# leggedrobotics/art_planner

Hardware: NVIDIA H100
Metric: pose-validity checks/s (higher is better)
Workload: dtype f32

## Files before the change

### art_planner_b200/capi.py

```python
from __future__ import annotations

import ctypes as C
import os

HERE = os.path.dirname(os.path.abspath(__file__))
LIB_PATH = os.path.join(HERE, "libartp.so")

ARTP_OK, ARTP_E_INVALID, ARTP_E_NOMAP, ARTP_E_CUDA, ARTP_E_LIMIT, ARTP_E_NOWEIGHTS, ARTP_E_WINDOW = 0, -1, -2, -3, -4, -5, -6


class ArtpError(RuntimeError):
    def __init__(self, code: int, msg: str):
        super().__init__(f"artp error {code}: {msg}")
        self.code = code


class ArtpParams(C.Structure):
    _fields_ = [(n, C.c_double) for n in (
        "torso_length", "torso_width", "torso_height", "torso_off_x", "torso_off_y", "torso_off_z",
        "feet_off_x", "feet_off_y", "feet_off_z", "reach_x", "reach_y", "reach_z")] + [
        ("unknown_space_untraversable", C.c_int), ("use_directional_cost", C.c_int),
        ("max_lon_vel", C.c_double), ("max_lat_vel", C.c_double), ("max_ang_vel", C.c_double),
        ("cost_w_energy", C.c_float), ("cost_w_time", C.c_float), ("cost_w_risk", C.c_float),
        ("risk_threshold", C.c_float), ("device", C.c_int)]
# ... 60 lines not shown
                ("sample_from_distribution", C.c_int), ("use_inverse_vertex_density", C.c_int),
                ("use_max_prob_unknown_samples", C.c_int), ("max_prob_unknown_samples", C.c_double), ("basic", ArtpBasicParams),
                ("simplify", C.c_int), ("clear_roadmap", C.c_int), ("seed", C.c_uint64)]


class ArtpPlanInfo(C.Structure):
    _fields_ = [("status", C.c_int32), ("sampled", C.c_int32)] + [(n, C.c_uint64) for n in (
        "first_sample", "draws_used", "start_draw", "goal_draw", "simplify_seed", "n_vertices", "n_edges")] + [
        ("solve", ArtpRoadmapSolveInfo), ("path_cost", C.c_double), ("simplify", ArtpSimplifyInfo)] + [
        (n, C.c_int32) for n in ("goal_clipped", "goal_inside", "start_index", "goal_index")] + [
        (n, C.c_double * 7) for n in ("goal_clipped_state", "goal_projected", "start_repaired", "goal_repaired")] + [
        (n, C.c_float) for n in ("ms_sample_graph", "ms_update_edges", "ms_endpoints", "ms_solve", "ms_simplify")] + [
        ("host_syncs", C.c_uint32), ("bytes_h2d", C.c_uint64), ("bytes_d2h", C.c_uint64)]


class ArtpPlannerMapInfo(C.Structure):
    _fields_ = [("host_syncs", C.c_uint32), ("bytes_h2d", C.c_uint64), ("bytes_d2h", C.c_uint64)]


class ArtpStats(C.Structure):
    _fields_ = [("poses_checked", C.c_uint64), ("poses_deferred", C.c_uint64), ("kernel_launches", C.c_uint64),
                ("last_deferred", C.c_uint32), ("last_launches", C.c_uint32), ("last_queued_boxes", C.c_uint32),
                ("last_queued_warp_stage", C.c_uint32), ("last_queued_reach_stage", C.c_uint32),
                ("last_reach_plane_stage", C.c_uint32)]


_lib = None


def load():
    global _lib
    if _lib is not None:
        return _lib
    if not os.path.exists(LIB_PATH):
        raise FileNotFoundError(f"{LIB_PATH} not built; run `python -m art_planner_b200.build` (needs nvcc)")
    lib = C.CDLL(LIB_PATH)
    vp, sz, i32, dbl = C.c_void_p, C.c_size_t, C.c_int, C.c_double
    lib.artp_create.argtypes = [C.POINTER(ArtpParams), C.POINTER(vp)]
    lib.artp_destroy.argtypes = [vp]
    lib.artp_destroy.restype = None
    lib.artp_last_error.argtypes = [vp]
    lib.artp_last_error.restype = C.c_char_p
    lib.artp_set_map.argtypes = [vp, vp, vp, i32, i32, dbl, dbl, dbl]
    lib.artp_has_map.argtypes = [vp]
    lib.artp_check_poses.argtypes = [vp, vp, sz, vp]
    lib.artp_check_poses_device.argtypes = [vp, vp, sz, vp, vp]
    lib.artp_check_poses_f32.argtypes = [vp, vp, sz, vp]
# ... 38 lines not shown
    lib.artp_update_sample_distribution_device.argtypes = [vp, C.POINTER(ArtpSampleDistributionParams), vp, sz, vp]
    lib.artp_debug_gaussian_kernel.argtypes = [i32, dbl, vp]
    lib.artp_roadmap_clear.argtypes = [vp, sz, sz]
    lib.artp_roadmap_add_milestones.argtypes = [vp, vp, sz]
    lib.artp_roadmap_sample_graph.argtypes = [vp, C.POINTER(ArtpRoadmapParams), C.POINTER(ArtpSampleDistributionParams), u64, u64,
                                              C.POINTER(u64)]
    lib.artp_roadmap_get.argtypes = [vp, sz, vp, vp, sz, vp, C.POINTER(sz), C.POINTER(sz)]
    lib.artp_roadmap_update_edges.argtypes = [vp]
    lib.artp_roadmap_solve.argtypes = [vp, vp, vp, C.POINTER(ArtpSe3Space), vp, sz, C.POINTER(sz), C.POINTER(dbl),
                                       C.POINTER(ArtpRoadmapSolveInfo)]
    lib.artp_roadmap_get_edge_costs.argtypes = [vp, sz, vp, vp, C.POINTER(sz)]
    lib.artp_debug_se3_ops.argtypes = [vp, vp, vp, vp, sz, vp, vp]
    lib.artp_simplify_path.argtypes = [vp, vp, sz, C.POINTER(ArtpSe3Space), i32, dbl, u64, vp, sz, C.POINTER(sz),
                                       C.POINTER(ArtpSimplifyInfo)]
    lib.artp_planner_set_map.argtypes = [vp, C.POINTER(ArtpPlannerParams), vp, vp, vp, vp, i32, i32, dbl, dbl, dbl,
                                         C.POINTER(ArtpPlannerMapInfo)]
    lib.artp_planner_get_space.argtypes = [vp, C.POINTER(ArtpSe3Space)]
    lib.artp_plan.argtypes = [vp, C.POINTER(ArtpPlannerParams), vp, vp, vp, sz, C.POINTER(sz), C.POINTER(ArtpPlanInfo)]
    lib.artp_host_alloc.restype = C.c_void_p
    lib.artp_host_alloc.argtypes = [sz]
    lib.artp_host_free.argtypes = [vp]
    lib.artp_debug_set_group_capacity.argtypes = [vp, i32]
    lib.artp_debug_get_reach_queue.argtypes = [vp, vp, sz, C.POINTER(sz)]
    lib.artp_set_timing.argtypes = [vp, i32]
    lib.artp_get_last_timing.argtypes = [vp, C.POINTER(C.c_float)]
    lib.artp_get_last_stage_timing.argtypes = [vp, C.POINTER(C.c_float)]
    lib.artp_version.restype = C.c_char_p
    lib.artp_cost_weights_size.restype = C.c_size_t
    lib.artp_cost_weights_size_for.restype = C.c_size_t
    lib.artp_cost_weights_size_for.argtypes = [i32]
    lib.artp_set_cost_weights.argtypes = [vp, vp, sz]
    lib.artp_get_cost_network.argtypes = [vp, C.POINTER(i32)]
    lib.artp_update_features.argtypes = [vp]
    lib.artp_motion_cost.argtypes = [vp, vp, sz, vp]
    lib.artp_motion_cost_device.argtypes = [vp, vp, sz, vp, vp]
    lib.artp_combine_cost.argtypes = [vp, vp, sz, vp, vp]
    lib.artp_motion_cost_split.argtypes = [vp, vp, vp, sz, dbl, vp]
    lib.artp_motion_cost_split_device.argtypes = [vp, vp, vp, sz, vp, sz, vp, vp, vp, vp]
    lib.artp_get_features.argtypes = [vp, vp, sz, C.POINTER(i32), C.POINTER(i32)]
    lib.artp_set_cnn_mode.argtypes = [vp, i32]
    lib.artp_get_cnn_timing.argtypes = [vp, C.POINTER(C.c_float)]
    _lib = lib
    return lib


def make_params(rp, device: int = 0, cost_weights=(0.0, 1.0, 5.0), risk_threshold=0.5) -> ArtpParams:
# ... 37 lines not shown
```

### art_planner_b200/checker.py

```python
from __future__ import annotations

import ctypes as C

import numpy as np

from . import capi


def _is_torch_cuda(x) -> bool:
    return hasattr(x, "is_cuda") and bool(x.is_cuda)


class _Handle:

    def __init__(self, robot_params, device: int = 0, cost_weights=(0.0, 1.0, 5.0), risk_threshold=0.5):
        self.lib = capi.load()
        self.params = robot_params
        self.device = device
        p = capi.make_params(robot_params, device, cost_weights, risk_threshold)
        h = C.c_void_p()
        rc = self.lib.artp_create(C.byref(p), C.byref(h))
        if rc != 0:
            raise capi.ArtpError(rc, self.lib.artp_last_error(None).decode())
        self.h = h
# ... 239 lines not shown
        if out_cnt is None:
            out_cnt = torch.empty(1, dtype=torch.int32, device=bits.device)
        self._h.check(self._h.lib.artp_compact_bits_device(self._h.h, C.c_void_p(bits.data_ptr()), n, int(base),
                                                           C.c_void_p(out_idx.data_ptr()), C.c_void_p(out_cnt.data_ptr()),
                                                           _stream_ptr()))
        return out_idx, out_cnt

    def setMode(self, mode: int) -> None:
        self._h.check(self._h.lib.artp_set_mode(self._h.h, int(mode)))

    def pollError(self) -> None:
        self._h.check(self._h.lib.artp_poll_error(self._h.h))

    def debugSetGroupCapacity(self, max_triangles: int) -> None:
        self._h.check(self._h.lib.artp_debug_set_group_capacity(self._h.h, int(max_triangles)))

    def debugReachQueue(self):
        import numpy as np
        n = C.c_size_t(0)
        self._h.check(self._h.lib.artp_debug_get_reach_queue(self._h.h, None, 0, C.byref(n)))
        buf = np.empty((n.value, 20), dtype=np.uint32)
        self._h.check(self._h.lib.artp_debug_get_reach_queue(self._h.h, C.c_void_p(buf.ctypes.data), n.value, C.byref(n)))
        return buf[:, 14:18].view(np.int32).copy(), buf[:, 19].copy()

    def stats(self) -> dict:
        return self._h.stats()

    def setTiming(self, enable: bool) -> None:
        self._h.check(self._h.lib.artp_set_timing(self._h.h, int(bool(enable))))

    def lastKernelTimesMs(self):
        ms = (C.c_float * 3)()
        self._h.check(self._h.lib.artp_get_last_timing(self._h.h, ms))
        return float(ms[0]), float(ms[1]), float(ms[2])

    def lastStageTimesMs(self):
        ms = (C.c_float * 5)()
        self._h.check(self._h.lib.artp_get_last_stage_timing(self._h.h, ms))
        return tuple(float(x) for x in ms)

    @property
    def handle(self) -> _Handle:
        return self._h


class SE3FromSE2Sampler:
# ... 579 lines not shown
```

### art_planner_b200/csrc/artp_capi.cu

```cuda
#include <cassert>
#include <climits>
#include <cmath>
#include <cstdlib>
#include <cstring>
#include <cudaTypedefs.h>
#include <type_traits>
#include <vector>

#include "artp_internal.h"
#include "artp_kernels.cuh"
#include "artp_tiles.cuh"

namespace artp_api {

constexpr int kMaxSlices = 9;

struct QueueCtr { uint32_t end, claim; };
struct alignas(32) BoxQueues { QueueCtr big, reach, group; };
struct Counters { BoxQueues q; uint32_t defer; };

struct Shape { int grid = 0, block = 0, smem = 0; };

struct Pipeline {
  enum { kBig, kReach, kGroup };
  Counters* d_ctr = nullptr;
  artp::BoxRec* recs[3] = {};
  uint32_t* d_defer = nullptr;
  size_t recs_cap = 0;
  BoxQueues* d_slices = nullptr;
  unsigned long long* d_compact_state = nullptr;
  size_t compact_state_cap = 0;
  uint32_t compact_epoch = 0;
  artp::TileCfg tile_cfg[2] = {};
  CUtensorMap tile_map[2][2];
  Shape tile[2];
  Shape groups;
  Shape grouping;
  int tcap = 0;
  int tcap_override = 0;
  int mode = 0;
  uint8_t* h_small_out = nullptr;
  bool deferred_unread = false;
  cudaStream_t streams[4] = {};
  cudaStream_t& copy_stream = streams[0];
  cudaStream_t& box_stream = streams[1];
  cudaStream_t& group_stream = streams[2];
  cudaStream_t& tile_stream = streams[3];
  cudaEvent_t order_ev[2 * kMaxSlices + 3] = {};
  cudaEvent_t *const copy_ev = order_ev, *const slice_ev = order_ev + kMaxSlices;
  cudaEvent_t& box_ev = order_ev[2 * kMaxSlices];
  cudaEvent_t &group_ev = order_ev[2 * kMaxSlices + 1], &tile_ev = order_ev[2 * kMaxSlices + 2];
// ... 279 lines not shown
  const size_t need = 5 * std::min(n_items, kChunkItems);
  if (h->pipe->recs_cap >= need) return ARTP_OK;
  const size_t cap = std::max<size_t>(need, 1u << 16);
  h->pipe->recs_cap = 0;
  for (artp::BoxRec*& r : h->pipe->recs) { size_t had = 0; TRY(grow(h, r, had, cap)); }
  size_t had = 0;
  TRY(grow(h, h->pipe->d_defer, had, cap));
  h->pipe->recs_cap = cap;
  return ARTP_OK;
}

struct HostFeed {
  const char* host;
  char* dev;
  size_t bytes_per_item;
  size_t slice_items;
  float schedule[8];
};
constexpr size_t kScheduleItems = 1u << 18;
constexpr int kPipeReachCtasPerSm = 2;

__global__ void close_slice_kernel(const BoxQueues* round, BoxQueues* slices, int i) {
  const BoxQueues prev = i ? slices[i - 1] : BoxQueues{};
  slices[i].group = {round->group.end, prev.group.end};
  slices[i].reach = {round->reach.end, prev.reach.end};
  slices[i].big = {round->big.end, prev.big.end};
}

artp::Work items(artp::Work w, size_t lo, size_t hi) {
  w.item_base = (uint32_t)lo;
  w.n_items = (uint32_t)hi;
  return w;
}
int launch_classify(Handle* h, const artp::Work& w, size_t lo, size_t hi, BoxQueues* q, cudaStream_t s) {
  const Pipeline& p = *h->pipe;
  return launch(h, artp::classify_items_kernel, (unsigned)((hi - lo + artp::kClassifyItems - 1) / artp::kClassifyItems),
                artp::kClassifyItems, 0, s, h->chk, items(w, lo, hi), p.recs[p.kBig], p.recs[p.kReach],
                p.groups.grid ? p.recs[p.kGroup] : nullptr, &q->big.end, &q->reach.end, &q->group.end, p.mode == 1);
}

int launch_big_tile(Handle* h, const artp::Work& w, size_t lo, size_t hi, BoxQueues* q, cudaStream_t s) {
  Pipeline& p = *h->pipe;
  const int wpc = p.tile[0].block / 32;
  const unsigned grid = (unsigned)std::min<size_t>((size_t)p.tile[0].grid, (5 * (hi - lo) + wpc - 1) / wpc);
  return launch(h, artp::box_tiles_warp_kernel, grid, p.tile[0].block, p.tile[0].smem, s, h->chk, p.tile_map[0][0],
                p.tile_map[0][1], p.tile_cfg[0], items(w, lo, hi), p.recs[p.kBig], &q->big.end, &q->big.claim, &p.d_ctr->defer,
                p.d_defer, 0u, p.mode == 1);
}
int launch_reach_warp(Handle* h, const artp::Work& w, size_t lo, size_t hi, BoxQueues* q, cudaStream_t s, unsigned reach_cap) {
  if (!h->chk.reach_tw) return ARTP_OK;
  Pipeline& p = *h->pipe;
  const int wpc = p.tile[1].block / 32;
  const unsigned grid = (unsigned)std::min<size_t>({(size_t)p.tile[1].grid, (4 * (hi - lo) + wpc - 1) / wpc, reach_cap});
  return launch(h, artp::box_tiles_warp_kernel, grid, p.tile[1].block, p.tile[1].smem, s, h->chk, p.tile_map[1][1],
                p.tile_map[1][1], p.tile_cfg[1], items(w, lo, hi), p.recs[p.kReach], &q->reach.end, &q->reach.claim,
                &p.d_ctr->defer, p.d_defer, artp::kDeferReachBit, p.mode == 1);
}
int launch_reach_groups(Handle* h, const artp::Work& w, size_t lo, size_t hi, BoxQueues* q, cudaStream_t s, unsigned reach_cap) {
  const Pipeline& p = *h->pipe;
  if (!p.groups.grid) return ARTP_OK;
  const unsigned grid = (unsigned)std::min<size_t>({(size_t)p.groups.grid, (hi - lo + 7) / 8, reach_cap});
  return launch(h, artp::reach_groups_kernel, grid, p.groups.block, p.groups.smem, s, h->chk, p.tile_map[1][1], p.tile_cfg[1],
                items(w, lo, hi), p.recs[p.kGroup], &q->group.end, &q->group.claim);
}

int launch_grouping(Handle* h, const artp::Work& w, size_t lo, size_t hi, cudaStream_t s) {
  const Pipeline& p = *h->pipe;
  const unsigned grid = (unsigned)std::min<size_t>((size_t)p.grouping.grid, 5 * (hi - lo));
  return launch(h, artp::box_items_block_kernel, grid, p.grouping.block, p.grouping.smem, s, h->chk, items(w, lo, hi),
                p.recs[p.kBig], p.recs[p.kReach], &p.d_ctr->defer, p.d_defer, p.tcap, h->d_err);
}

int run_round_device(Handle* h, const artp::Work& w, cudaStream_t s, size_t base, size_t end, bool timed) {
  Pipeline& p = *h->pipe;
  CU_TRY(h, cudaMemsetAsync(p.d_ctr, 0, sizeof(Counters), s));
  if (timed) CU_TRY(h, cudaEventRecord(p.ev[0], s));
  BoxQueues* q = &p.d_ctr->q;
  TRY(launch_classify(h, w, base, end, q, s));
  if (timed) CU_TRY(h, cudaEventRecord(p.ev[1], s));
  const bool fork = !p.timing && h->chk.reach_tw;
  if (fork) {
    CU_TRY(h, cudaEventRecord(p.slice_ev[0], s));
    CU_TRY(h, cudaStreamWaitEvent(p.tile_stream, p.slice_ev[0], 0));
    CU_TRY(h, cudaStreamWaitEvent(p.box_stream, p.slice_ev[0], 0));
    if (p.groups.grid) CU_TRY(h, cudaStreamWaitEvent(p.group_stream, p.slice_ev[0], 0));
  }
// ... 451 lines not shown
  LOCK_HANDLE(h, hh);
  return timed_round_ms(h, ms5, {{0, 1}, {1, 2}, {2, 3}, {3, 4}, {4, 5}});
}

void* artp_host_alloc(size_t bytes) {
  void* p = nullptr;
  if (bytes == 0 || cudaHostAlloc(&p, bytes, cudaHostAllocPortable) != cudaSuccess) return nullptr;
  return p;
}
void artp_host_free(void* p) { if (p) cudaFreeHost(p); }

int artp_poll_error(artp_handle* hh) {
  LOCK_HANDLE(h, hh);
  return take_sticky_error(h);
}

int artp_debug_set_group_capacity(artp_handle* hh, int max_triangles) {
  LOCK_HANDLE(h, hh);
  if (max_triangles < 0) return ARTP_E_INVALID;
  h->pipe->tcap_override = max_triangles;
  return ARTP_OK;
}

int artp_debug_get_reach_queue(artp_handle* hh, void* recs, size_t cap, size_t* n) {
  LOCK_HANDLE(h, hh);
  if (!n || (cap && !recs)) return ARTP_E_INVALID;
  CU_TRY(h, cudaSetDevice(h->device));
  Counters ctr{};
  CU_TRY(h, cudaMemcpy(&ctr, h->pipe->d_ctr, sizeof(ctr), cudaMemcpyDeviceToHost));
  *n = ctr.q.reach.end;
  const size_t k = std::min(cap, (size_t)ctr.q.reach.end);
  if (k) CU_TRY(h, cudaMemcpy(recs, h->pipe->recs[h->pipe->kReach], k * sizeof(artp::BoxRec), cudaMemcpyDeviceToHost));
  return ARTP_OK;
}

int artp_get_stats(artp_handle* hh, artp_stats* out) {
  LOCK_HANDLE(h, hh);
  if (!out) return ARTP_E_INVALID;
  CU_TRY(h, cudaSetDevice(h->device));
  Counters ctr{};
  CU_TRY(h, cudaMemcpy(&ctr, h->pipe->d_ctr, sizeof(ctr), cudaMemcpyDeviceToHost));
  h->stats.last_deferred = ctr.defer;
  h->stats.last_queued_boxes = ctr.q.big.end + ctr.q.reach.end + ctr.q.group.end;
  h->stats.last_queued_warp_stage = ctr.q.big.end;
  h->stats.last_queued_reach_stage = ctr.q.reach.end;
  h->stats.last_reach_plane_stage = ctr.q.group.end;
  if (h->pipe->deferred_unread) { h->stats.poses_deferred += ctr.defer; h->pipe->deferred_unread = false; }
  *out = h->stats;
  return take_sticky_error(h);
}

int artp_set_map(artp_handle* hh, const float* elevation, const float* elevation_masked, int rows, int cols, double res,
                 double cx, double cy) {
  return artp_set_map_window(hh, elevation, elevation_masked, rows, cols, res, cx, cy, 0, rows);
}

int artp_set_map_window(artp_handle* hh, const float* elevation, const float* elevation_masked, int rows, int cols, double res,
                        double cx, double cy, int row0, int nrows) {
  LOCK_CALL(h, hh);
  h->planner_map = false;
  return upload_map(h, elevation, elevation_masked, false, rows, cols, res, cx, cy, row0, nrows);
}

}

int artp_api::upload_map(Handle* h, const float* elevation, const float* elevation_masked, bool device_src, int rows, int cols,
                         double res, double cx, double cy, int row0, int nrows) {
  if (!elevation || !elevation_masked || rows < 2 || cols < 2 || !(res > 0)) { h->err = "bad map arguments"; return ARTP_E_INVALID; }
  if (row0 < 0 || nrows < 2 || row0 + nrows > rows || (row0 & 3)) {
// ... 278 lines not shown
```

### art_planner_b200/csrc/artp_kernels.cuh

```cuda
#pragma once

#include "artp_device.cuh"

namespace artp {

constexpr int kWarpsPerCta = 8;
constexpr int kMaxCand = 32;
constexpr int kBloomWords = 128;
constexpr unsigned kFull = 0xffffffffu;

enum { R_FREE = 0, R_HIT = 1, R_DEFER = 2 };

__device__ __forceinline__ bool box_fails(bool foot, int r) { return foot ? r == R_FREE : r == R_HIT; }

struct WarpScratch {
  float cpl[kMaxCand][4];
  int cidx[kMaxCand];
  uint32_t bloom[kBloomWords];
  uint32_t bloom2[kBloomWords];
  uint32_t cand_bits[kBloomWords];
};

struct Work {
  const double* s1 = nullptr;
// ... 650 lines not shown
  fl = (uint32_t)k;
  const int g = box_geometry(c, R, R1, t, k, b);
  if (g != -1) return g;
  const int r = zone_classify(c, b, k, force_all, fl);
  return (r == -1 && probe_applies(b, fl) && vertex_probe(c, b, k > 0)) ? R_HIT : r;
}

constexpr int kClassifyItems = 64;
constexpr int kClassifyWarps = kClassifyItems / 32;
constexpr int kPoseWords = 21;
enum { PEND_BIG = 1, PEND_REACH = 2, PEND_GROUP = 3 };

struct ClassifyShared {
  float pose[kPoseWords][kClassifyItems];
  float probe_f[4][kClassifyItems];
  int probe_i[4][kClassifyItems];
  uint8_t valid[kClassifyItems];
  uint8_t pend[5][kClassifyItems];
  uint16_t live[kClassifyItems];
  uint16_t probe[kClassifyItems];
  uint16_t emit[5 * kClassifyItems];
  unsigned long long warp_sum[kClassifyWarps];
  int warp_count[kClassifyWarps];
  uint32_t base[3];
};
static_assert(kClassifyItems <= 256, "emit packs the item index into 8 bits");

__device__ __forceinline__ void load_pose(const ClassifyShared& s, int i, float t[3], float R[9], float R1[9]) {
#pragma unroll
  for (int j = 0; j < 3; ++j) t[j] = s.pose[j][i];
#pragma unroll
  for (int j = 0; j < 9; ++j) { R[j] = s.pose[3 + j][i]; R1[j] = s.pose[12 + j][i]; }
}

__device__ __forceinline__ unsigned long long cta_scan(ClassifyShared& s, unsigned long long v, unsigned long long& total) {
  const int lane = threadIdx.x & 31, wid = threadIdx.x >> 5;
  unsigned long long incl = v;
#pragma unroll
  for (int o = 1; o < 32; o <<= 1) {
    const unsigned long long y = __shfl_up_sync(kFull, incl, o);
    if (lane >= o) incl += y;
  }
  if (lane == 31) s.warp_sum[wid] = incl;
  __syncthreads();
  unsigned long long before = 0;
  total = 0;
#pragma unroll
  for (int q = 0; q < kClassifyWarps; ++q) {
    const unsigned long long x = s.warp_sum[q];
// ... 2 lines not shown
  }
  return before + incl - v;
}

__device__ __forceinline__ int cta_compact(ClassifyShared& s, uint16_t* list, bool pred, int entry) {
  const int lane = threadIdx.x & 31, wid = threadIdx.x >> 5;
  const unsigned m = __ballot_sync(kFull, pred);
  if (lane == 0) s.warp_count[wid] = __popc(m);
  __syncthreads();
  int before = 0, total = 0;
#pragma unroll
  for (int q = 0; q < kClassifyWarps; ++q) {
    const int x = s.warp_count[q];
    before += q < wid ? x : 0;
    total += x;
  }
  if (pred) list[before + __popc(m & ((1u << lane) - 1u))] = (uint16_t)entry;
  __syncthreads();
  return total;
}

__global__ void __launch_bounds__(kClassifyItems, 16)
classify_items_kernel(const Checker c, const Work w, BoxRec* __restrict__ recs_w, BoxRec* __restrict__ recs_f,
                      BoxRec* __restrict__ recs_g, uint32_t* __restrict__ count_w, uint32_t* __restrict__ count_f,
                      uint32_t* __restrict__ count_g, int force_all) {
  __shared__ ClassifyShared s;
  const int tid = threadIdx.x;
  const uint32_t item0 = w.item_base + blockIdx.x * kClassifyItems;
  const bool in_range = item0 + tid < w.n_items;
  if (in_range) {
    double st[7];
    load_item_state(w, item0 + tid, st);
    float t[3], R[9], Rb[9];
    pose3_from_se3(st, t, R);
#pragma unroll
    for (int i = 0; i < 9; ++i) Rb[i] = R[i];
    orthogonalize_r(Rb);
#pragma unroll
    for (int j = 0; j < 3; ++j) s.pose[j][tid] = t[j];
#pragma unroll
    for (int j = 0; j < 9; ++j) s.pose[3 + j][tid] = R[j];
#pragma unroll
    for (int j = 0; j < 3; ++j) { s.pose[12 + j][tid] = -Rb[j]; s.pose[15 + j][tid] = Rb[6 + j]; s.pose[18 + j][tid] = Rb[3 + j]; }
  }
  s.valid[tid] = in_range ? 1 : 0;
#pragma unroll
  for (int k = 0; k < 5; ++k) s.pend[k][tid] = 0;

// ... 29 lines not shown
    if (!foot) break;
    const int n_probe = cta_compact(s, s.probe, probe, tid);
    if (tid < n_probe) {
      const int p = s.probe[tid], i = s.live[p];
      BoxCtx b;
      b.P[0] = s.probe_f[0][p]; b.P[1] = s.probe_f[1][p]; b.P[2] = s.probe_f[2][p]; b.minB = s.probe_f[3][p];
      b.x0 = s.probe_i[0][p]; b.x1 = s.probe_i[1][p]; b.z0 = s.probe_i[2][p]; b.z1 = s.probe_i[3][p];
#pragma unroll
      for (int j = 0; j < 9; ++j) b.R1[j] = s.pose[12 + j][i];
      b.side[0] = c.side[1][0]; b.side[1] = c.side[1][1]; b.side[2] = c.side[1][2];
      if (vertex_probe(c, b, true)) s.pend[k][i] = 0;
    }
  }
  __syncthreads();

  const bool valid = s.valid[tid] != 0;
  if (in_range) {
    const uint32_t slot = item_slot(w, item0 + tid);
    if (w.edge_mode) { if (!valid) w.valid[slot] = 0; }
    else w.valid[slot] = (uint8_t)valid;
  }
  unsigned long long cnt = 0;
  if (valid) {
#pragma unroll
    for (int k = 0; k < 5; ++k) {
      const int q = s.pend[k][tid] >> 6;
      if (q) cnt += 1ull << (21 * (q - 1));
    }
  }
  unsigned long long tot;
  unsigned long long off = cta_scan(s, cnt, tot);
  if (tot == 0) return;
  const uint32_t n_w = (uint32_t)(tot & 0x1FFFFF), n_f = (uint32_t)((tot >> 21) & 0x1FFFFF), n_g = (uint32_t)(tot >> 42);
  if (tid == 0) {
    s.base[0] = n_w ? atomicAdd(count_w, n_w) : 0u;
    s.base[1] = n_f ? atomicAdd(count_f, n_f) : 0u;
    s.base[2] = n_g ? atomicAdd(count_g, n_g) : 0u;
  }
  if (cnt) {
    uint32_t pw = (uint32_t)(off & 0x1FFFFF), pf = n_w + (uint32_t)((off >> 21) & 0x1FFFFF), pg = n_w + n_f + (uint32_t)(off >> 42);
#pragma unroll
    for (int k = 0; k < 5; ++k) {
      const int q = s.pend[k][tid] >> 6;
      const uint16_t e = (uint16_t)((k << 8) | tid);
      if (q == PEND_BIG) s.emit[pw++] = e;
      else if (q == PEND_REACH) s.emit[pf++] = e;
      else if (q == PEND_GROUP) s.emit[pg++] = e;
    }
  }
  __syncthreads();
  const uint32_t n_rec = n_w + n_f + n_g;
#pragma unroll 1
  for (uint32_t j = tid; j < n_rec; j += kClassifyItems) {
    const int e = s.emit[j], i = e & 0xFF, k = e >> 8;
    float t[3], R[9], R1[9];
    load_pose(s, i, t, R, R1);
    BoxCtx b;
    box_geometry(c, R, R1, t, k, b);
    BoxRec o;
#pragma unroll
    for (int m = 0; m < 9; ++m) o.R1[m] = R1[m];
    o.P[0] = b.P[0]; o.P[1] = b.P[1]; o.P[2] = b.P[2];
    o.minB = b.minB; o.maxB = b.maxB;
    o.x0 = b.x0; o.x1 = b.x1; o.z0 = b.z0; o.z1 = b.z1;
    o.item = item_slot(w, item0 + i);
    o.flags = s.pend[k][i] & 0x3Fu;
    if (j < n_w) recs_w[s.base[0] + j] = o;
    else if (j < n_w + n_f) recs_f[s.base[1] + (j - n_w)] = o;
    else recs_g[s.base[2] + (j - n_w - n_f)] = o;
  }
}

struct BlockShared {
  float* planes;
  int* group;
  uint8_t* state;
  int T_cap;
};
__device__ __forceinline__ BlockShared block_shared(unsigned char* smem, int T_cap) {
  BlockShared sh;
  sh.T_cap = T_cap;
  sh.planes = reinterpret_cast<float*>(smem);
  sh.group = reinterpret_cast<int*>(smem + (size_t)T_cap * 16);
  sh.state = reinterpret_cast<uint8_t*>(smem + (size_t)T_cap * 20);
  return sh;
}

__device__ __forceinline__ float block_reduce_max(float v, float* red, bool is_max) {
  const int lane = threadIdx.x & 31, wid = threadIdx.x >> 5;
#pragma unroll
  for (int o = 16; o > 0; o >>= 1) {
    const float a = __shfl_xor_sync(kFull, v, o);
// ... 245 lines not shown
```

### art_planner_b200/csrc/artp_tiles.cuh

```cuda
#pragma once

#include <cuda.h>

#include "artp_kernels.cuh"

namespace artp {

constexpr uint32_t kDeferReachBit = 0x80000000u;
constexpr int kTileChunk = 8;

__device__ __forceinline__ uint32_t smem_addr(const void* p) { return (uint32_t)__cvta_generic_to_shared(p); }
__device__ __forceinline__ void mbar_init(uint64_t* bar, uint32_t count) {
  asm volatile("mbarrier.init.shared::cta.b64 [%0], %1;" ::"r"(smem_addr(bar)), "r"(count));
}
__device__ __forceinline__ void mbar_expect_tx(uint64_t* bar, uint32_t bytes) {
  asm volatile("mbarrier.arrive.expect_tx.shared::cta.b64 _, [%0], %1;" ::"r"(smem_addr(bar)), "r"(bytes) : "memory");
}
__device__ __forceinline__ void mbar_wait(uint64_t* bar, uint32_t parity) {
  asm volatile(
      "{\n\t"
      ".reg .pred P1;\n\t"
      "TWAIT_LOOP:\n\t"
      "mbarrier.try_wait.parity.shared::cta.b64 P1, [%0], %1;\n\t"
      "@P1 bra TWAIT_DONE;\n\t"
// ... 81 lines not shown
      phase[slot] ^= 1u;
      if (dead) continue;
      BoxCtx b;
      rec_to_ctx(c, r, b);
      int res;
      if ((b.x1 - b.x0) + 4 > tc.tw || (b.z1 - b.z0) + 1 > tc.th) {
        res = R_DEFER;
      } else {
        const ZoneView zv{reinterpret_cast<const float*>(slots + (size_t)slot * tc.stride) + (b.x0 & 3), tc.tw};
        res = box_collide_warp<true>(foot ? c.f[1] : c.f[0], b, zv, ws, lane, c.cell_margin, (r.flags & REC_NEEDS_REDUCE) != 0,
                                     (r.flags & REC_ALLFINITE) != 0, (r.flags & REC_MERGEFREE) != 0);
      }
      if (lane == 0) {
        if (res == R_DEFER) defer_list[atomicAdd(defer_count, 1u)] = ri | queue_bit;
        else if (box_fails(foot, res)) w.valid[slot_item] = 0;
      }
    }
  }
}

constexpr int kGroupRounds = 8;
constexpr int kGroupTasks = 64;

__global__ void __launch_bounds__(kMaxTileWarps * 32, 3)
reach_groups_kernel(const Checker c, const __grid_constant__ CUtensorMap map1, const TileCfg tc, const Work w,
                    const BoxRec* __restrict__ recs, const uint32_t* __restrict__ rec_count, uint32_t* __restrict__ work_counter) {
  extern __shared__ __align__(128) unsigned char tile_smem[];
  __shared__ uint64_t bars[kMaxTileWarps][2];
  __shared__ uint16_t tasks_all[kMaxTileWarps][4][kGroupTasks];
  __shared__ __align__(16) float ctx_all[kMaxTileWarps][4][16];
  const int lane = threadIdx.x & 31, wid = threadIdx.x >> 5, g = lane >> 3, gl = lane & 7;
  const Field& f = c.f[1];
  unsigned char* slots = warp_tile_slots(tile_smem, tc, 8, bars[wid]);
  uint16_t* tasks = tasks_all[wid][g];
  uint32_t phase = 0u;
  const uint32_t total = *rec_count;
  const unsigned gshift = (unsigned)g * 8u;
  auto prefetch = [&](uint32_t first, int slot) {
    const uint32_t ri = first + (uint32_t)g;
    int x0 = 0, z0 = 0;
    const bool act = ri < total;
    if (act && gl == 0) { x0 = rec_x0(recs + ri); z0 = rec_z0(recs + ri); }
    const int nact = (int)min(4u, total - first);
    if (lane == 0) mbar_expect_tx(&bars[wid][slot], (uint32_t)nact * tc.bytes);
#pragma unroll 1
    for (int q = 0; q < nact; ++q) {
      const int sx = __shfl_sync(kFull, x0, q * 8), sz = __shfl_sync(kFull, z0, q * 8);
      if (lane == 0) tma_tile_2d(slots + (size_t)(slot * 4 + q) * tc.stride, &map1, &bars[wid][slot], (sx & ~3) - tc.x_off, sz);
    }
  };
  const uint32_t nwarps8 = 8u * gridDim.x * (blockDim.x >> 5);
  uint32_t next_r0 = 0, next_n = 0;
  auto claim = [&]() {
    if (lane == 0) {
      const uint32_t cur = *(volatile const uint32_t*)work_counter;
      next_n = 4u * (cur < total ? min(max((total - cur) / nwarps8, 1u), (uint32_t)kGroupRounds) : 1u);
      next_r0 = atomicAdd(work_counter, next_n);
    }
  };
  claim();
  for (;;) {
    const uint32_t r0 = __shfl_sync(kFull, next_r0, 0), nclaim = __shfl_sync(kFull, next_n, 0);
    if (r0 >= total) break;
    claim();
    const int nrounds = (int)((min(r0 + nclaim, total) - r0 + 3u) / 4u);
    __syncwarp();
    prefetch(r0, 0);
#pragma unroll 1
    for (int round = 0; round < nrounds; ++round) {
      const int slot = round & 1;
      const uint32_t ri = r0 + 4u * (uint32_t)round + (uint32_t)g;
      const bool act = ri < total;
      BoxRec r = {};
      if (act) r = load_rec(recs + ri);
      if (round + 1 < nrounds) { __syncwarp(); prefetch(r0 + 4u * (uint32_t)(round + 1), slot ^ 1); }
      int alive = 0;
      if (act && gl == 0) alive = (*(volatile const uint8_t*)(w.valid + r.item) != 0);
      alive = __shfl_sync(kFull, alive, 0, 8);
      mbar_wait(&bars[wid][slot], (phase >> slot) & 1u);
      phase ^= 1u << slot;
      __syncwarp();
      bool gdone = !(act && alive);
      BoxCtx b;
      rec_to_ctx(c, r, b);
      if (gdone) { b.x0 = b.z0 = 0; b.x1 = b.z1 = 1; }
      if (gl == 0) {
        float* cx = ctx_all[wid][g];
#pragma unroll
        for (int i = 0; i < 9; ++i) cx[i] = b.R1[i];
        cx[9] = b.P[0]; cx[10] = b.P[1]; cx[11] = b.P[2]; cx[12] = b.minB;
        cx[13] = __int_as_float(b.x0); cx[14] = __int_as_float(b.z0);
      }
      const float* tile = reinterpret_cast<const float*>(slots + (size_t)(slot * 4 + g) * tc.stride) + (b.x0 & 3);
      const float top = b.maxB + (1e-4f + 4e-6f * fabsf(b.maxB));
      bool ghit = false;
      const bool allFinite = (r.flags & REC_ALLFINITE) != 0;
      {
        const float xr = box_half_extent(b.R1, b.side, 0) + 1e-4f, zr = box_half_extent(b.R1, b.side, 2) + 1e-4f;
        const int vx0 = max(b.x0, (int)ceilf((b.P[0] - xr) * f.iW)), vx1 = min(b.x1, (int)floorf((b.P[0] + xr) * f.iW));
        const int vz0 = max(b.z0, (int)ceilf((b.P[2] - zr) * f.iD)), vz1 = min(b.z1, (int)floorf((b.P[2] + zr) * f.iD));
        const int nXi = max(vx1 - vx0 + 1, 0), nZi = max(vz1 - vz0 + 1, 0), nVi = nXi * nZi;
// ... 73 lines not shown
            const int lx = tk >> 9, lz = (tk >> 1) & 0xff, ccx = tx0 + lx, ccz = tz0 + lz;
            const float* p = reinterpret_cast<const float*>(slots + (size_t)(slot * 4 + gi) * tc.stride) + (tx0 & 3) + lz * tc.tw + lx;
            const float hA = p[0], hB = p[1], hC = p[tc.tw], hD = p[tc.tw + 1];
            if (tri_kept(isUp, hA, hB, hC, hD, tb.minB)) {
              float pl[4], cxs[4], czs[4];
              cell_plane(f, isUp, ccx, ccz, hA, hB, hC, hD, pl);
              const int nc = box_plane(tb, pl, 4, cxs, czs);
              const int tcx = isUp ? ccx : ccx + 1, tcz = isUp ? ccz : ccz + 1;
              bool hit = false;
#pragma unroll
              for (int i = 0; i < 4; ++i) hit = hit || (i < nc && on_tri(f, isUp, tcx, tcz, cxs[i], czs[i]));
              if (hit) hit_groups |= 1u << gi;
            }
          }
        }
        __syncwarp();
        hit_groups = __reduce_or_sync(kFull, hit_groups);
        if ((hit_groups >> g) & 1u) ghit = true;
      }
      if (gl == 0 && act && alive && box_fails(true, ghit ? R_HIT : R_FREE)) w.valid[r.item] = 0;
      __syncwarp();
    }
  }
}

}
```

### include/artp.h

```cpp
#ifndef ARTP_H
#define ARTP_H

#include <stddef.h>
#include <stdint.h>

#ifdef __cplusplus
extern "C" {
#endif

#define ARTP_OK            0
#define ARTP_E_INVALID    -1
#define ARTP_E_NOMAP      -2
#define ARTP_E_CUDA       -3
#define ARTP_E_LIMIT      -4
#define ARTP_E_NOWEIGHTS  -5
#define ARTP_E_WINDOW     -6

typedef struct artp_params {
  double torso_length, torso_width, torso_height;
  double torso_off_x, torso_off_y, torso_off_z;
  double feet_off_x, feet_off_y, feet_off_z;
  double reach_x, reach_y, reach_z;
  int    unknown_space_untraversable;
  int    use_directional_cost;
  double max_lon_vel, max_lat_vel, max_ang_vel;
  float  cost_w_energy, cost_w_time, cost_w_risk;
  float  risk_threshold;
  int    device;
} artp_params;

typedef struct artp_handle artp_handle;

typedef struct artp_stats {
  uint64_t poses_checked;
  uint64_t poses_deferred;
  uint64_t kernel_launches;
  uint32_t last_deferred;
  uint32_t last_launches;
  uint32_t last_queued_boxes;
  uint32_t last_queued_warp_stage;
  uint32_t last_queued_reach_stage;
  uint32_t last_reach_plane_stage;
} artp_stats;

int  artp_create(const artp_params* params, artp_handle** out);
void artp_destroy(artp_handle* h);
const char* artp_last_error(const artp_handle* h);

int artp_set_map(artp_handle* h, const float* elevation, const float* elevation_masked,
                 int rows, int cols, double res, double cx, double cy);
int artp_has_map(const artp_handle* h);
int artp_set_map_window(artp_handle* h, const float* elevation, const float* elevation_masked, int rows, int cols,
                        double res, double cx, double cy, int row0, int nrows);

int artp_check_poses(artp_handle* h, const double* states, size_t n, uint8_t* valid);
int artp_check_poses_device(artp_handle* h, const double* d_states, size_t n, uint8_t* d_valid, void* stream);

void* artp_host_alloc(size_t bytes);
void  artp_host_free(void* p);

int artp_check_poses_f32(artp_handle* h, const float* states, size_t n, uint8_t* valid);
int artp_check_poses_f32_device(artp_handle* h, const float* d_states, size_t n, uint8_t* d_valid, void* stream);

int artp_check_motions(artp_handle* h, const double* s1, const double* s2, size_t n, int n_steps, uint8_t* valid);
int artp_check_motions_device(artp_handle* h, const double* d_s1, const double* d_s2, size_t n, int n_steps,
// ... 42 lines not shown
                                int32_t* d_index, void* stream);
int artp_ball_offsets(artp_handle* h, uint64_t seed, uint64_t first_draw, size_t n, uint32_t n_iter, const double* radius,
                      double* offsets);
int artp_pose_from_2d(artp_handle* h, const double* states_in, size_t n, double* states_out, uint8_t* inside);

int artp_path_length_cost(artp_handle* h, const double* s1, const double* s2, size_t n, double* cost);
int artp_path_length_cost_device(artp_handle* h, const double* d_s1, const double* d_s2, size_t n,
                                 double* d_cost, void* stream);

int artp_compact_valid_device(artp_handle* h, const uint8_t* d_valid, size_t n, int64_t base,
                              int64_t* d_indices, uint32_t* d_count, void* stream);
int artp_pack_valid_bits_device(artp_handle* h, const uint8_t* d_valid, size_t n, uint32_t* d_bits, void* stream);
int artp_check_poses_bits_device(artp_handle* h, const double* d_states, size_t n, uint8_t* d_valid, uint32_t* d_bits, void* stream);
int artp_compact_valid_u32_device(artp_handle* h, const uint8_t* d_valid, size_t n, uint32_t base, uint32_t* d_indices,
                                  uint32_t* d_count, void* stream);
int artp_compact_bits_device(artp_handle* h, const uint32_t* d_bits, size_t n, int64_t base, int64_t* d_indices,
                             uint32_t* d_count, void* stream);

int artp_get_stats(artp_handle* h, artp_stats* out);

int artp_poll_error(artp_handle* h);
int artp_debug_set_group_capacity(artp_handle* h, int max_triangles);
int artp_debug_get_reach_queue(artp_handle* h, void* recs, size_t cap, size_t* n);


int artp_set_timing(artp_handle* h, int enable);
int artp_get_last_timing(artp_handle* h, float* ms3);
int artp_get_last_stage_timing(artp_handle* h, float* ms5);

int artp_set_mode(artp_handle* h, int mode);

typedef struct artp_basic_params {
  float  traversability_thres;
  int    unknown_space_untraversable;
  double foothold_margin, foothold_margin_max_hole_size, foothold_margin_max_drop,
         foothold_margin_max_drop_search_radius, foothold_margin_min_step, foothold_size;
} artp_basic_params;
int artp_process_basic(artp_handle* h, const float* elevation, const float* traversability, const float* observed, int rows,
                       int cols, double res, const artp_basic_params* bp, float* elevation_masked, float* traversability_thresholded);
int artp_debug_circular_kernel(int size, uint8_t* out);

typedef struct artp_sample_distribution_params {
  int    use_inverse_vertex_density;
  double density_blur_radius;
  int    use_max_prob_unknown_samples;
  double max_prob_unknown_samples;
// ... 148 lines not shown
```

### profiles/reach_rounds.py

```python
import argparse
import json
import os
import subprocess
import sys
import tempfile

ROOT = os.path.dirname(os.path.dirname(os.path.abspath(__file__)))
sys.path.insert(0, ROOT)

import numpy as np
import torch

import art_planner_b200 as ap
from art_planner_b200 import synth
import bench

STAGES = ("classify", "torso_queue", "reach_queue_warp", "reach_queue_groups", "group")


def card():
    q = subprocess.run(["nvidia-smi", "--query-gpu=name,power.limit,clocks.max.sm", "--format=csv,noheader", "-i",
                        str(torch.cuda.current_device())], capture_output=True, text=True)
    name, power, clock = (x.strip() for x in (q.stdout.strip().split(",") + ["", "", ""])[:3])
    return {"name": name, "power_limit": power, "max_sm_clock": clock}
# ... 18 lines not shown
    chk.setMap(m)
    chk.updateHeightField()
    chk.setTiming(True)
    d_poses = torch.from_numpy(poses).cuda()
    d_valid = torch.empty(n, dtype=torch.uint8, device="cuda")
    flush = torch.empty(256 * 1024 * 1024, dtype=torch.uint8, device="cuda")
    sms = torch.cuda.get_device_properties(0).multi_processor_count

    for i in range(args.warmup):
        flush.fill_(i % 255 + 1)
        chk.isValidBatch(d_poses, out=d_valid)
    torch.cuda.synchronize()
    times = []
    for i in range(args.steps):
        flush.fill_(i % 255 + 1)
        chk.isValidBatch(d_poses, out=d_valid)
        times.append(chk.lastStageTimesMs())
        torch.cuda.synchronize()
    st = chk.stats()
    t = np.array(times, dtype=np.float64)
    med = dict(zip(STAGES, (round(float(x), 5) for x in np.median(t, 0))))
    spread = dict(zip(STAGES, (round(float(x), 5) for x in np.percentile(t, 90, 0) - np.percentile(t, 10, 0))))
    q_warp, q_groups = st["last_queued_reach_stage"], st["last_reach_plane_stage"]

    with torch.profiler.profile(activities=[torch.profiler.ProfilerActivity.CUDA]) as prof:
        for i in range(3):
            chk.isValidBatch(d_poses, out=d_valid)
        torch.cuda.synchronize()
    raw = os.path.join(args.out or tempfile.mkdtemp(), "reach_rounds.pt.trace.json")
    os.makedirs(os.path.dirname(raw), exist_ok=True)
    prof.export_chrome_trace(raw)
    with open(raw) as f:
        evs = [e for e in json.load(f)["traceEvents"] if e.get("ph") == "X" and e.get("cat") == "kernel"]
    evs.sort(key=lambda e: e["ts"])
    tiles = [e for e in evs if "box_tiles_warp_kernel" in e["name"]]
    groups = [e for e in evs if "reach_groups_kernel" in e["name"]]
    grid_warp = tiles[1]["args"]["grid"][0] if len(tiles) > 1 else None
    grid_groups = groups[0]["args"]["grid"][0] if groups else None

    ms_w, ms_g = med["reach_queue_warp"], med["reach_queue_groups"]
    res = {
        "card": card(), "workload": "c2_rough" if args.rough else "configs[1]", "sms": sms, "steps": args.steps, "stage_ms_median": med, "stage_ms_p90_minus_p10": spread,
        "reach_warp": {"queued_boxes": q_warp, "ms": ms_w, "grid": grid_warp,
                       "ctas_per_sm": grid_warp / sms if grid_warp else None,
                       "boxes_per_s_per_sm": q_warp / (ms_w * 1e-3) / sms if ms_w > 0 else None},
        "reach_groups": {"queued_boxes": q_groups, "rounds": (q_groups + 3) // 4, "ms": ms_g, "grid": grid_groups,
                         "ctas_per_sm": grid_groups / sms if grid_groups else None,
                         "rounds_per_s_per_sm": (q_groups + 3) // 4 / (ms_g * 1e-3) / sms if ms_g > 0 else None},
    }
    line = json.dumps(res)
    print(line)
    if args.out:
        with open(os.path.join(args.out, "reach_rounds.json"), "w") as f:
            f.write(line + "\n")
        os.remove(raw)


if __name__ == "__main__":
    main()
```

Measured before the change: 2.084 billion.

## Split reach-group queue into two tiers and skip records of already-invalid poses

The classify kernel now puts a pose's first group-stage box in a tier-1 queue and its later boxes in a separate tier-2 region, both counted with one packed 64-bit atomic. The reach_groups kernel walks tier 1 first, then tier 2, and filters each claimed batch by the pose's current validity flag, so boxes of poses already rejected are never prefetched or tested. Per-queue counters shrink from 21-bit to 16-bit fields, and a 'decided' counter plus a debug queue readout are added for profiling. Risks: extra validity loads and ballot work per claim, and the tier-2 region is placed at a fixed offset of capacity/5 that could overflow.

```diff
diff --git a/art_planner_b200/capi.py b/art_planner_b200/capi.py
--- a/art_planner_b200/capi.py
+++ b/art_planner_b200/capi.py
@@ -106,7 +106,7 @@
     _fields_ = [("poses_checked", C.c_uint64), ("poses_deferred", C.c_uint64), ("kernel_launches", C.c_uint64),
                 ("last_deferred", C.c_uint32), ("last_launches", C.c_uint32), ("last_queued_boxes", C.c_uint32),
                 ("last_queued_warp_stage", C.c_uint32), ("last_queued_reach_stage", C.c_uint32),
-                ("last_reach_plane_stage", C.c_uint32)]
+                ("last_reach_plane_stage", C.c_uint32), ("last_reach_plane_decided", C.c_uint32)]
 
 
 _lib = None
@@ -191,6 +191,7 @@
     lib.artp_host_free.argtypes = [vp]
     lib.artp_debug_set_group_capacity.argtypes = [vp, i32]
     lib.artp_debug_get_reach_queue.argtypes = [vp, vp, sz, C.POINTER(sz)]
+    lib.artp_debug_get_box_queue.argtypes = [vp, C.c_int, vp, sz, C.POINTER(sz)]
     lib.artp_set_timing.argtypes = [vp, i32]
     lib.artp_get_last_timing.argtypes = [vp, C.POINTER(C.c_float)]
     lib.artp_get_last_stage_timing.argtypes = [vp, C.POINTER(C.c_float)]
diff --git a/art_planner_b200/checker.py b/art_planner_b200/checker.py
--- a/art_planner_b200/checker.py
+++ b/art_planner_b200/checker.py
@@ -285,6 +285,15 @@
         buf = np.empty((n.value, 20), dtype=np.uint32)
         self._h.check(self._h.lib.artp_debug_get_reach_queue(self._h.h, C.c_void_p(buf.ctypes.data), n.value, C.byref(n)))
         return buf[:, 14:18].view(np.int32).copy(), buf[:, 19].copy()
+
+    def debugBoxQueue(self, queue: int):
+        import numpy as np
+        n = C.c_size_t(0)
+        self._h.check(self._h.lib.artp_debug_get_box_queue(self._h.h, int(queue), None, 0, C.byref(n)))
+        buf = np.empty((n.value, 20), dtype=np.uint32)
+        self._h.check(self._h.lib.artp_debug_get_box_queue(self._h.h, int(queue), C.c_void_p(buf.ctypes.data), n.value,
+                                                           C.byref(n)))
+        return buf
 
     def stats(self) -> dict:
         return self._h.stats()
diff --git a/art_planner_b200/csrc/artp_capi.cu b/art_planner_b200/csrc/artp_capi.cu
--- a/art_planner_b200/csrc/artp_capi.cu
+++ b/art_planner_b200/csrc/artp_capi.cu
@@ -16,8 +16,9 @@
 constexpr int kMaxSlices = 9;
 
 struct QueueCtr { uint32_t end, claim; };
-struct alignas(32) BoxQueues { QueueCtr big, reach, group; };
-struct Counters { BoxQueues q; uint32_t defer; };
+struct alignas(32) BoxQueues { QueueCtr big, reach; artp::GroupQueue group; };
+static_assert(sizeof(BoxQueues) == 32, "one sector per slice");
+struct Counters { BoxQueues q; uint32_t defer; alignas(128) uint32_t group_decided; };
 
 struct Shape { int grid = 0, block = 0, smem = 0; };
 
@@ -27,6 +28,7 @@
   artp::BoxRec* recs[3] = {};
   uint32_t* d_defer = nullptr;
   size_t recs_cap = 0;
+  uint32_t tier2_at() const { return (uint32_t)(recs_cap / 5); }
   BoxQueues* d_slices = nullptr;
   unsigned long long* d_compact_state = nullptr;
   size_t compact_state_cap = 0;
@@ -352,7 +354,7 @@
 
 __global__ void close_slice_kernel(const BoxQueues* round, BoxQueues* slices, int i) {
   const BoxQueues prev = i ? slices[i - 1] : BoxQueues{};
-  slices[i].group = {round->group.end, prev.group.end};
+  slices[i].group = {round->group.end1, round->group.end2, prev.group.end1, prev.group.end2};
   slices[i].reach = {round->reach.end, prev.reach.end};
   slices[i].big = {round->big.end, prev.big.end};
 }
@@ -366,7 +368,8 @@
   const Pipeline& p = *h->pipe;
   return launch(h, artp::classify_items_kernel, (unsigned)((hi - lo + artp::kClassifyItems - 1) / artp::kClassifyItems),
                 artp::kClassifyItems, 0, s, h->chk, items(w, lo, hi), p.recs[p.kBig], p.recs[p.kReach],
-                p.groups.grid ? p.recs[p.kGroup] : nullptr, &q->big.end, &q->reach.end, &q->group.end, p.mode == 1);
+                p.groups.grid ? p.recs[p.kGroup] : nullptr, p.groups.grid ? p.recs[p.kGroup] + p.tier2_at() : nullptr,
+                &q->big.end, &q->reach.end, reinterpret_cast<unsigned long long*>(&q->group.end1), p.mode == 1);
 }
 
 int launch_big_tile(Handle* h, const artp::Work& w, size_t lo, size_t hi, BoxQueues* q, cudaStream_t s) {
@@ -391,7 +394,7 @@
   if (!p.groups.grid) return ARTP_OK;
   const unsigned grid = (unsigned)std::min<size_t>({(size_t)p.groups.grid, (hi - lo + 7) / 8, reach_cap});
   return launch(h, artp::reach_groups_kernel, grid, p.groups.block, p.groups.smem, s, h->chk, p.tile_map[1][1], p.tile_cfg[1],
-                items(w, lo, hi), p.recs[p.kGroup], &q->group.end, &q->group.claim);
+                items(w, lo, hi), p.recs[p.kGroup], p.tier2_at(), &q->group, &p.d_ctr->group_decided);
 }
 
 int launch_grouping(Handle* h, const artp::Work& w, size_t lo, size_t hi, cudaStream_t s) {
@@ -889,16 +892,23 @@
   return ARTP_OK;
 }
 
+int artp_debug_get_box_queue(artp_handle* hh, int queue, void* recs, size_t cap, size_t* n) {
+  LOCK_HANDLE(h, hh);
+  if (!n || (cap && !recs) || queue < 0 || queue > 2) return ARTP_E_INVALID;
+  CU_TRY(h, cudaSetDevice(h->device));
+  const Pipeline& p = *h->pipe;
+  Counters ctr{};
+  CU_TRY(h, cudaMemcpy(&ctr, p.d_ctr, sizeof(ctr), cudaMemcpyDeviceToHost));
+  const uint32_t len[3] = {ctr.q.reach.end, ctr.q.group.end1, ctr.q.group.end2};
+  const artp::BoxRec* src[3] = {p.recs[p.kReach], p.recs[p.kGroup], p.recs[p.kGroup] + p.tier2_at()};
+  *n = len[queue];
+  const size_t k = std::min(cap, (size_t)len[queue]);
+  if (k) CU_TRY(h, cudaMemcpy(recs, src[queue], k * sizeof(artp::BoxRec), cudaMemcpyDeviceToHost));
+  return ARTP_OK;
+}
+
 int artp_debug_get_reach_queue(artp_handle* hh, void* recs, size_t cap, size_t* n) {
-  LOCK_HANDLE(h, hh);
-  if (!n || (cap && !recs)) return ARTP_E_INVALID;
-  CU_TRY(h, cudaSetDevice(h->device));
-  Counters ctr{};
-  CU_TRY(h, cudaMemcpy(&ctr, h->pipe->d_ctr, sizeof(ctr), cudaMemcpyDeviceToHost));
-  *n = ctr.q.reach.end;
-  const size_t k = std::min(cap, (size_t)ctr.q.reach.end);
-  if (k) CU_TRY(h, cudaMemcpy(recs, h->pipe->recs[h->pipe->kReach], k * sizeof(artp::BoxRec), cudaMemcpyDeviceToHost));
-  return ARTP_OK;
+  return artp_debug_get_box_queue(hh, 0, recs, cap, n);
 }
 
 int artp_get_stats(artp_handle* hh, artp_stats* out) {
@@ -908,10 +918,11 @@
   Counters ctr{};
   CU_TRY(h, cudaMemcpy(&ctr, h->pipe->d_ctr, sizeof(ctr), cudaMemcpyDeviceToHost));
   h->stats.last_deferred = ctr.defer;
-  h->stats.last_queued_boxes = ctr.q.big.end + ctr.q.reach.end + ctr.q.group.end;
+  h->stats.last_queued_boxes = ctr.q.big.end + ctr.q.reach.end + ctr.q.group.end1 + ctr.q.group.end2;
   h->stats.last_queued_warp_stage = ctr.q.big.end;
   h->stats.last_queued_reach_stage = ctr.q.reach.end;
-  h->stats.last_reach_plane_stage = ctr.q.group.end;
+  h->stats.last_reach_plane_stage = ctr.q.group.end1 + ctr.q.group.end2;
+  h->stats.last_reach_plane_decided = ctr.group_decided;
   if (h->pipe->deferred_unread) { h->stats.poses_deferred += ctr.defer; h->pipe->deferred_unread = false; }
   *out = h->stats;
   return take_sticky_error(h);
diff --git a/art_planner_b200/csrc/artp_kernels.cuh b/art_planner_b200/csrc/artp_kernels.cuh
--- a/art_planner_b200/csrc/artp_kernels.cuh
+++ b/art_planner_b200/csrc/artp_kernels.cuh
@@ -696,9 +696,10 @@
   uint16_t emit[5 * kClassifyItems];
   unsigned long long warp_sum[kClassifyWarps];
   int warp_count[kClassifyWarps];
-  uint32_t base[3];
+  uint32_t base[4];
 };
 static_assert(kClassifyItems <= 256, "emit packs the item index into 8 bits");
+static_assert(5 * kClassifyItems < (1 << 16), "a CTA's record count per queue is a 16-bit field of the emission scan");
 
 __device__ __forceinline__ void load_pose(const ClassifyShared& s, int i, float t[3], float R[9], float R1[9]) {
 #pragma unroll
@@ -747,8 +748,9 @@
 
 __global__ void __launch_bounds__(kClassifyItems, 16)
 classify_items_kernel(const Checker c, const Work w, BoxRec* __restrict__ recs_w, BoxRec* __restrict__ recs_f,
-                      BoxRec* __restrict__ recs_g, uint32_t* __restrict__ count_w, uint32_t* __restrict__ count_f,
-                      uint32_t* __restrict__ count_g, int force_all) {
+                      BoxRec* __restrict__ recs_g, BoxRec* __restrict__ recs_g2, uint32_t* __restrict__ count_w,
+                      uint32_t* __restrict__ count_f, unsigned long long* __restrict__ count_g2,
+                      int force_all) {
   __shared__ ClassifyShared s;
   const int tid = threadIdx.x;
   const uint32_t item0 = w.item_base + blockIdx.x * kClassifyItems;
@@ -824,34 +826,41 @@
   }
   unsigned long long cnt = 0;
   if (valid) {
+    int tier = 0;
 #pragma unroll
     for (int k = 0; k < 5; ++k) {
       const int q = s.pend[k][tid] >> 6;
-      if (q) cnt += 1ull << (21 * (q - 1));
+      if (q) cnt += 1ull << (16 * (q - 1 + (q == PEND_GROUP ? tier : 0)));
+      if (q == PEND_GROUP) tier = 1;
     }
   }
   unsigned long long tot;
   unsigned long long off = cta_scan(s, cnt, tot);
   if (tot == 0) return;
-  const uint32_t n_w = (uint32_t)(tot & 0x1FFFFF), n_f = (uint32_t)((tot >> 21) & 0x1FFFFF), n_g = (uint32_t)(tot >> 42);
+  const uint32_t n_w = (uint32_t)(tot & 0xFFFF), n_f = (uint32_t)((tot >> 16) & 0xFFFF), n_g = (uint32_t)((tot >> 32) & 0xFFFF),
+                 n_g2 = (uint32_t)(tot >> 48);
   if (tid == 0) {
     s.base[0] = n_w ? atomicAdd(count_w, n_w) : 0u;
     s.base[1] = n_f ? atomicAdd(count_f, n_f) : 0u;
-    s.base[2] = n_g ? atomicAdd(count_g, n_g) : 0u;
+    const unsigned long long g = (n_g || n_g2) ? atomicAdd(count_g2, n_g | (unsigned long long)n_g2 << 32) : 0ull;
+    s.base[2] = (uint32_t)g;
+    s.base[3] = (uint32_t)(g >> 32);
   }
   if (cnt) {
-    uint32_t pw = (uint32_t)(off & 0x1FFFFF), pf = n_w + (uint32_t)((off >> 21) & 0x1FFFFF), pg = n_w + n_f + (uint32_t)(off >> 42);
+    uint32_t pw = (uint32_t)(off & 0xFFFF), pf = n_w + (uint32_t)((off >> 16) & 0xFFFF);
+    uint32_t pg = n_w + n_f + (uint32_t)((off >> 32) & 0xFFFF), pg2 = n_w + n_f + n_g + (uint32_t)(off >> 48);
+    bool tier1 = true;
 #pragma unroll
     for (int k = 0; k < 5; ++k) {
       const int q = s.pend[k][tid] >> 6;
       const uint16_t e = (uint16_t)((k << 8) | tid);
       if (q == PEND_BIG) s.emit[pw++] = e;
       else if (q == PEND_REACH) s.emit[pf++] = e;
-      else if (q == PEND_GROUP) s.emit[pg++] = e;
+      else if (q == PEND_GROUP) { if (tier1) s.emit[pg++] = e; else s.emit[pg2++] = e; tier1 = false; }
     }
   }
   __syncthreads();
-  const uint32_t n_rec = n_w + n_f + n_g;
+  const uint32_t n_rec = n_w + n_f + n_g + n_g2;
 #pragma unroll 1
   for (uint32_t j = tid; j < n_rec; j += kClassifyItems) {
     const int e = s.emit[j], i = e & 0xFF, k = e >> 8;
@@ -869,7 +878,8 @@
     o.flags = s.pend[k][i] & 0x3Fu;
     if (j < n_w) recs_w[s.base[0] + j] = o;
     else if (j < n_w + n_f) recs_f[s.base[1] + (j - n_w)] = o;
-    else recs_g[s.base[2] + (j - n_w - n_f)] = o;
+    else if (j < n_w + n_f + n_g) recs_g[s.base[2] + (j - n_w - n_f)] = o;
+    else recs_g2[s.base[3] + (j - n_w - n_f - n_g)] = o;
   }
 }
 
diff --git a/art_planner_b200/csrc/artp_tiles.cuh b/art_planner_b200/csrc/artp_tiles.cuh
--- a/art_planner_b200/csrc/artp_tiles.cuh
+++ b/art_planner_b200/csrc/artp_tiles.cuh
@@ -127,26 +127,32 @@
 constexpr int kGroupRounds = 8;
 constexpr int kGroupTasks = 64;
 
+struct alignas(8) GroupQueue { uint32_t end1, end2, claim, begin2; };
+static_assert(offsetof(GroupQueue, end2) == offsetof(GroupQueue, end1) + 4, "the two tier ends are one 64-bit word");
+
 __global__ void __launch_bounds__(kMaxTileWarps * 32, 3)
 reach_groups_kernel(const Checker c, const __grid_constant__ CUtensorMap map1, const TileCfg tc, const Work w,
-                    const BoxRec* __restrict__ recs, const uint32_t* __restrict__ rec_count, uint32_t* __restrict__ work_counter) {
+                    const BoxRec* __restrict__ recs, uint32_t tier2_at, GroupQueue* __restrict__ queue,
+                    uint32_t* __restrict__ decided) {
   extern __shared__ __align__(128) unsigned char tile_smem[];
   __shared__ uint64_t bars[kMaxTileWarps][2];
   __shared__ uint16_t tasks_all[kMaxTileWarps][4][kGroupTasks];
   __shared__ __align__(16) float ctx_all[kMaxTileWarps][4][16];
+  __shared__ uint32_t live_all[kMaxTileWarps][4 * kGroupRounds];
   const int lane = threadIdx.x & 31, wid = threadIdx.x >> 5, g = lane >> 3, gl = lane & 7;
   const Field& f = c.f[1];
   unsigned char* slots = warp_tile_slots(tile_smem, tc, 8, bars[wid]);
   uint16_t* tasks = tasks_all[wid][g];
+  const uint32_t* live = live_all[wid];
   uint32_t phase = 0u;
-  const uint32_t total = *rec_count;
+  const uint32_t end1 = queue->end1, shift2 = tier2_at + queue->begin2 - end1, total = end1 + (queue->end2 - queue->begin2);
+  uint32_t* const work_counter = &queue->claim;
   const unsigned gshift = (unsigned)g * 8u;
-  auto prefetch = [&](uint32_t first, int slot) {
-    const uint32_t ri = first + (uint32_t)g;
+  int nlive = 0;
+  auto prefetch = [&](int first, int slot) {
     int x0 = 0, z0 = 0;
-    const bool act = ri < total;
-    if (act && gl == 0) { x0 = rec_x0(recs + ri); z0 = rec_z0(recs + ri); }
-    const int nact = (int)min(4u, total - first);
+    if (first + g < nlive && gl == 0) { const uint32_t ri = live[first + g]; x0 = rec_x0(recs + ri); z0 = rec_z0(recs + ri); }
+    const int nact = min(4, nlive - first);
     if (lane == 0) mbar_expect_tx(&bars[wid][slot], (uint32_t)nact * tc.bytes);
 #pragma unroll 1
     for (int q = 0; q < nact; ++q) {
@@ -163,25 +169,38 @@
       next_r0 = atomicAdd(work_counter, next_n);
     }
   };
+  uint32_t ndecided = 0;
   claim();
   for (;;) {
     const uint32_t r0 = __shfl_sync(kFull, next_r0, 0), nclaim = __shfl_sync(kFull, next_n, 0);
     if (r0 >= total) break;
     claim();
-    const int nrounds = (int)((min(r0 + nclaim, total) - r0 + 3u) / 4u);
-    __syncwarp();
-    prefetch(r0, 0);
+    {
+      const uint32_t v = r0 + (uint32_t)lane;
+      const uint32_t ri = v < end1 ? v : v + shift2;
+      const bool act = (uint32_t)lane < nclaim && v < total;
+      bool lv = false;
+      if (act) lv = *(volatile const uint8_t*)(w.valid + rec_field(recs + ri, offsetof(BoxRec, item))) != 0;
+      const unsigned lm = __ballot_sync(kFull, lv);
+      __syncwarp();
+      if (lv) live_all[wid][__popc(lm & ((1u << lane) - 1u))] = ri;
+      nlive = __popc(lm);
+      __syncwarp();
+    }
+    const int nrounds = (nlive + 3) / 4;
+    if (nrounds) prefetch(0, 0);
 #pragma unroll 1
     for (int round = 0; round < nrounds; ++round) {
       const int slot = round & 1;
-      const uint32_t ri = r0 + 4u * (uint32_t)round + (uint32_t)g;
-      const bool act = ri < total;
+      const int li = 4 * round + g;
+      const bool act = li < nlive;
       BoxRec r = {};
-      if (act) r = load_rec(recs + ri);
-      if (round + 1 < nrounds) { __syncwarp(); prefetch(r0 + 4u * (uint32_t)(round + 1), slot ^ 1); }
+      if (act) r = load_rec(recs + live[li]);
+      if (round + 1 < nrounds) { __syncwarp(); prefetch(4 * (round + 1), slot ^ 1); }
       int alive = 0;
       if (act && gl == 0) alive = (*(volatile const uint8_t*)(w.valid + r.item) != 0);
       alive = __shfl_sync(kFull, alive, 0, 8);
+      ndecided += __popc(__ballot_sync(kFull, gl == 0 && alive));
       mbar_wait(&bars[wid][slot], (phase >> slot) & 1u);
       phase ^= 1u << slot;
       __syncwarp();
@@ -301,6 +320,7 @@
       __syncwarp();
     }
   }
-}
-
-}
+  if (lane == 0 && ndecided) atomicAdd(decided, ndecided);
+}
+
+}
diff --git a/include/artp.h b/include/artp.h
--- a/include/artp.h
+++ b/include/artp.h
@@ -41,6 +41,7 @@
   uint32_t last_queued_warp_stage;
   uint32_t last_queued_reach_stage;
   uint32_t last_reach_plane_stage;
+  uint32_t last_reach_plane_decided;
 } artp_stats;
 
 int  artp_create(const artp_params* params, artp_handle** out);
@@ -129,6 +130,7 @@
 int artp_poll_error(artp_handle* h);
 int artp_debug_set_group_capacity(artp_handle* h, int max_triangles);
 int artp_debug_get_reach_queue(artp_handle* h, void* recs, size_t cap, size_t* n);
+int artp_debug_get_box_queue(artp_handle* h, int queue, void* recs, size_t cap, size_t* n);
 
 
 int artp_set_timing(artp_handle* h, int enable);
diff --git a/profiles/reach_rounds.py b/profiles/reach_rounds.py
--- a/profiles/reach_rounds.py
+++ b/profiles/reach_rounds.py
@@ -64,6 +64,8 @@
     med = dict(zip(STAGES, (round(float(x), 5) for x in np.median(t, 0))))
     spread = dict(zip(STAGES, (round(float(x), 5) for x in np.percentile(t, 90, 0) - np.percentile(t, 10, 0))))
     q_warp, q_groups = st["last_queued_reach_stage"], st["last_reach_plane_stage"]
+    tier1, tier2 = len(chk.debugBoxQueue(1)), len(chk.debugBoxQueue(2))
+    decided = st["last_reach_plane_decided"]
 
     with torch.profiler.profile(activities=[torch.profiler.ProfilerActivity.CUDA]) as prof:
         for i in range(3):
@@ -86,7 +88,9 @@
         "reach_warp": {"queued_boxes": q_warp, "ms": ms_w, "grid": grid_warp,
                        "ctas_per_sm": grid_warp / sms if grid_warp else None,
                        "boxes_per_s_per_sm": q_warp / (ms_w * 1e-3) / sms if ms_w > 0 else None},
-        "reach_groups": {"queued_boxes": q_groups, "rounds": (q_groups + 3) // 4, "ms": ms_g, "grid": grid_groups,
+        "reach_groups": {"queued_boxes": q_groups, "tier1": tier1, "tier2": tier2, "decided": decided,
+                         "skipped": q_groups - decided, "skipped_share": round((q_groups - decided) / q_groups, 4) if q_groups else None,
+                         "rounds": (q_groups + 3) // 4, "ms": ms_g, "grid": grid_groups,
                          "ctas_per_sm": grid_groups / sms if grid_groups else None,
                          "rounds_per_s_per_sm": (q_groups + 3) // 4 / (ms_g * 1e-3) / sms if ms_g > 0 else None},
     }
```

Result: no change. 2.081 billion (median of 6 runs) (-0.1%).
